# microsoft/ORBIT-Dataset

Measured on AMD Instinct MI355X. Metric: query frames/sec per task (224×224, 5-way ProtoNet) + frame accuracy vs ref, higher is better.
Workload: dtype f32

## Files before the change

### include/orbit_hip.h

```cpp
#ifndef ORBIT_HIP_H
#define ORBIT_HIP_H

#include <stddef.h>
#include <stdint.h>

#ifdef __cplusplus
extern "C" {
#endif

typedef struct orbit_extractor orbit_extractor_t;
typedef struct orbit_filmgen orbit_filmgen_t;
typedef struct orbit_vit orbit_vit_t;
typedef void* orbit_stream_t;

#define ORBIT_OK 0
#define ORBIT_ERR_ARG (-1)
#define ORBIT_ERR_HIP (-2)
#define ORBIT_ERR_STATE (-3)
#define ORBIT_ERR_NOMEM (-4)

#define ORBIT_ACT_NONE 0
#define ORBIT_ACT_RELU 1
#define ORBIT_ACT_SILU 2
#define ORBIT_ACT_ELU 3
// ... 121 lines not shown
int orbit_pw_stream_supported(int Cin, int Cout, int H, int W);
int orbit_op_dwconv2d(const float* x, const float* w, float* y, const float* scale, const float* shift,
                      int B, int H, int W, int C, int K, int stride, int pad_top, int pad_left,
                      int Ho, int Wo, int act, orbit_stream_t stream);
int orbit_op_conv2d_train(const float* x, int x_nchw, const float* w, float* y, const float* gate, int B, int H, int W,
                          int Cin, int Cout, int KH, int KW, int stride, int pad_top, int pad_left, int Ho, int Wo,
                          float* stats, int* stat_blocks, orbit_stream_t stream);
int orbit_op_conv2d_plan(int B, int H, int W, int Cin, int Cout, int KH, int KW, int stride, int pad_top, int pad_left, int Ho, int Wo,
                         int x_nchw, int pool2, int gated, int residual, int flags, int stats_mode, int dual_output, char* row,
                         int* ksplit, int* kt_per_split, int* m_tiles);
int orbit_op_conv2d_plan_ex(int B, int H, int W, int Cin, int Cout, int KH, int KW, int stride, int pad_top, int pad_left, int Ho,
                            int Wo, int x_nchw, int pool2, int gated, int residual, int flags, int stats_mode, int dual_output, int act,
                            char* row, int* ksplit, int* kt_per_split, int* m_tiles, int* epilogue);
int orbit_op_dwconv2d_train(const float* x, const float* w, float* y, const float* in_scale, const float* in_shift,
                            int in_act, int B, int H, int W, int C, int K, int stride, int pad_top, int pad_left, int Ho,
                            int Wo, float* stats, orbit_stream_t stream);
int orbit_op_dwconv2d_se(const float* x, const float* w, const float* scale, const float* shift, int act, int B, int H, int W,
                         int C, int K, int stride, int pad_top, int pad_left, int Ho, int Wo, float* y, float* partial,
                         orbit_stream_t stream);
int orbit_op_dwconv2d_plan(int B, int C, int K, int stride, int Ho, int Wo, int train_form, int* form, int* chunks,
                           int* rows_per_chunk);
int orbit_op_se_gate2(const float* partial, int chunks, int hw, const float* w1, const float* b1, const float* w2,
                      const float* b2, int B, int C, int R, float* gate, float* pooled_out, orbit_stream_t stream);
int orbit_op_maxpool2d(const float* x, float* y, int B, int H, int W, int C, int K, int stride, int pad,
                       int Ho, int Wo, orbit_stream_t stream);
int orbit_op_avgpool(const float* x, float* y, int B, int HW, int C, orbit_stream_t stream);
int orbit_op_se_gate(const float* pooled, const float* w1, const float* b1, const float* w2,
                     const float* b2, float* gate, int B, int C, int R, orbit_stream_t stream);

int orbit_op_vit_linear(const float* x, const float* w, const float* bias, const float* residual, float* y, int M, int N,
                        int K, int epilogue, int tile_rows, orbit_stream_t stream);
int orbit_op_vit_patch_embed(const float* frames, const float* w, const float* bias_or_null, const float* pos_embed,
                             const float* cls_token, float* tokens, int B, int D, int tile_rows, orbit_stream_t stream);
int orbit_op_vit_patch_embed_p(const float* frames, const float* w, const float* bias_or_null, const float* pos_embed,
                               const float* cls_token, float* tokens, int B, int D, int patch, int tile_rows,
                               orbit_stream_t stream);
int orbit_op_vit_layernorm(const float* x, size_t x_stride, float* y, size_t y_stride, int rows, int D, const float* gamma,
                           const float* beta, float eps, orbit_stream_t stream);
int orbit_op_vit_attention(const float* qkv, float* out, int B, int D, int heads, orbit_stream_t stream);
int orbit_op_vit_attention_tokens(const float* qkv, float* out, int B, int tokens, int D, int heads, orbit_stream_t stream);
int orbit_op_vit_linear_dgrad(const float* dy, const float* w, float* wt_scratch, const float* u, const float* residual,
                              float* dx, int M, int N, int K, int tile_rows, orbit_stream_t stream);
int orbit_op_vit_layernorm_bwd(const float* x, size_t x_stride, const float* dy, size_t dy_stride, const float* gamma, float eps,
                               const float* dres, float* dx, size_t dx_stride, int rows, int D, float* dgamma, float* dbeta,
                               float* partial, size_t partial_floats, orbit_stream_t stream);
int orbit_op_vit_attention_bwd(const float* qkv, const float* dout, float* dqkv, int B, int D, int heads,
// ... 278 lines not shown
```

### orbit-dataset_amd/_lib.py

```python
import ctypes
import os
from ctypes import c_char_p, c_double, c_float, c_int, c_size_t, c_void_p, POINTER

_HERE = os.path.dirname(os.path.abspath(__file__))
LIB_PATH = os.path.join(_HERE, "lib", "liborbit_hip.so")

_lib = None

P = c_void_p
_SIGNATURES = {
    "orbit_version": (c_int, []),
    "orbit_last_error": (c_char_p, []),
    "orbit_device_count": (c_int, []),
    "orbit_set_option": (c_int, [c_char_p, c_int]),
    "orbit_get_option": (c_int, [c_char_p]),
    "orbit_label_set": (c_int, [P, c_int, P, c_int, P, P]),
    "orbit_proto_configure": (c_int, [P, P, P, c_int, c_int, c_int, c_int, c_int, P, P, P]),
    "orbit_proto_finalize": (c_int, [P, P, c_int, c_int, c_int, c_int, P, P, P]),
    "orbit_proto_predict": (c_int, [P, P, P, c_int, c_int, c_int, c_int, c_int, c_float, c_int, P, P, P]),
    "orbit_video_metrics": (c_int, [P, c_int, c_int, P, P, c_int, P, P, P, P, P]),
    "orbit_mean_pool": (c_int, [P, c_int, c_int, c_int, P, P]),
    "orbit_set_mean": (c_int, [P, c_int, c_int, P, P]),
    "orbit_history_mean_pool": (c_int, [P, c_int, c_int, c_int, P, P]),
    "orbit_extractor_create": (c_int, [c_char_p, c_int, c_int, POINTER(c_void_p)]),
# ... 38 lines not shown
    "orbit_vit_backward": (c_int, [P, c_int, P, P, P, P, c_size_t, P, P, P, c_size_t, P]),
    "orbit_vit_grad_floats": (c_size_t, [P]),
    "orbit_vit_param_offset": (c_size_t, [P, c_int]),
    "orbit_vit_backward_params_workspace_bytes": (c_size_t, [P, c_int]),
    "orbit_vit_backward_params": (c_int, [P, P, c_int, P, P, P, P, c_size_t, P, P, P, P, c_size_t, P]),
    "orbit_filmgen_create": (c_int, [c_int, c_int, c_int, POINTER(c_int), POINTER(c_int), POINTER(c_int),
                                     POINTER(c_void_p)]),
    "orbit_filmgen_destroy": (None, [P]),
    "orbit_filmgen_load": (c_int, [P, c_int, c_char_p, P, c_size_t]),
    "orbit_filmgen_load_all_async": (c_int, [P, P, c_int, P]),
    "orbit_filmgen_forward": (c_int, [P, P, P, P, P, P]),
    "orbit_op_conv2d": (c_int, [P, c_int, P, P, P, P, P, P] + [c_int] * 14 + [P]),
    "orbit_op_conv2d_ex": (c_int, [P, c_int, P, P, P, P, P, P] + [c_int] * 15 + [P]),
    "orbit_op_dwconv2d": (c_int, [P, P, P, P, P] + [c_int] * 11 + [P]),
    "orbit_op_pw_stream": (c_int, [P] * 6 + [c_int] + [P] * 4 + [c_int, P, P] + [c_int] * 5 + [P]),
    "orbit_pw_stream_supported": (c_int, [c_int] * 4),
    "orbit_op_conv2d_train": (c_int, [P, c_int, P, P, P] + [c_int] * 12 + [P, POINTER(c_int), P]),
    "orbit_op_conv2d_plan": (c_int, [c_int] * 19 + [c_char_p] + [POINTER(c_int)] * 3),
    "orbit_op_conv2d_plan_ex": (c_int, [c_int] * 20 + [c_char_p] + [POINTER(c_int)] * 4),
    "orbit_op_dwconv2d_train": (c_int, [P, P, P, P, P] + [c_int] * 11 + [P, P]),
    "orbit_op_dwconv2d_se": (c_int, [P, P, P, P] + [c_int] * 11 + [P, P, P]),
    "orbit_op_dwconv2d_plan": (c_int, [c_int] * 7 + [POINTER(c_int)] * 3),
    "orbit_op_se_gate2": (c_int, [P, c_int, c_int, P, P, P, P, c_int, c_int, c_int, P, P, P]),
    "orbit_op_maxpool2d": (c_int, [P, P] + [c_int] * 9 + [P]),
    "orbit_op_avgpool": (c_int, [P, P, c_int, c_int, c_int, P]),
    "orbit_op_se_gate": (c_int, [P, P, P, P, P, P, c_int, c_int, c_int, P]),
    "orbit_op_vit_linear": (c_int, [P] * 5 + [c_int] * 5 + [P]),
    "orbit_op_vit_patch_embed": (c_int, [P] * 6 + [c_int] * 3 + [P]),
    "orbit_op_vit_layernorm": (c_int, [P, c_size_t, P, c_size_t, c_int, c_int, P, P, c_float, P]),
    "orbit_op_vit_attention": (c_int, [P, P, c_int, c_int, c_int, P]),
    "orbit_op_vit_attention_tokens": (c_int, [P, P, c_int, c_int, c_int, c_int, P]),
    "orbit_op_vit_patch_embed_p": (c_int, [P] * 6 + [c_int] * 4 + [P]),
    "orbit_op_vit_linear_dgrad": (c_int, [P] * 6 + [c_int] * 4 + [P]),
    "orbit_op_vit_layernorm_bwd": (c_int, [P, c_size_t, P, c_size_t, P, c_float, P, P, c_size_t, c_int, c_int, P, P, P,
                                           c_size_t, P]),
    "orbit_op_vit_attention_bwd": (c_int, [P, P, P, c_int, c_int, c_int, P]),
    "orbit_op_vit_attention_bwd_tokens": (c_int, [P, P, P, c_int, c_int, c_int, c_int, P]),
    "orbit_op_vit_linear_wgrad_workspace_floats": (c_size_t, [c_int, c_int, c_int]),
    "orbit_op_vit_linear_wgrad": (c_int, [P] * 4 + [c_int] * 4 + [P, c_size_t, P]),
    "orbit_op_vit_patch_embed_bwd": (c_int, [P] * 6 + [c_int] * 2 + [P, c_size_t, P]),
    "orbit_op_mbconv_front": (c_int, [P] * 9 + [c_int] * 11 + [P]),
    "orbit_op_mbconv_front_partials": (c_int, [c_int] * 6),
    "orbit_op_stem_dw_front_partials": (c_int, [c_int] * 3),
    "orbit_op_stem_dw_front": (c_int, [P] * 9 + [c_int] * 12 + [P]),
    "orbit_dense_rows": (c_int, [P, c_int, c_int, P, P, c_int, c_int, P, P, P]),
    "orbit_spd_inverse": (c_int, [P, P, c_int, c_int, P]),
# ... 242 lines not shown
```

### orbit-dataset_amd/csrc/common.h

```cpp
#pragma once
#include <hip/hip_runtime.h>
#include <cstdarg>
#include <cstdio>
#include <cstdint>
#include <cstring>
#include <type_traits>
#include "../../include/orbit_hip.h"

namespace orbit {

char* err_buf();
int set_err(int code, const char* fmt, ...);
int get_option(const char* name);
int option_epoch();

#define ORBIT_HIP_CHECK(expr)                                                                  \
    do {                                                                                       \
        hipError_t _e = (expr);                                                                \
        if (_e != hipSuccess)                                                                  \
            return ::orbit::set_err(ORBIT_ERR_HIP, "%s failed: %s (%s:%d)", #expr,             \
                                    hipGetErrorString(_e), __FILE__, __LINE__);                \
    } while (0)

#define ORBIT_LAUNCH_CHECK()                                                                   \
// ... 175 lines not shown
    int form = 0, chunks = 0, rpc = 0, bn_rows = 0, wgrad_rows = 0;
};
DwBwdForm dwconv_se_bwd_form(const LayerGeom& g, bool want_wgrad);
template <class F>
static inline void dw_dispatch_ks(int K, int stride, F&& f) {
    using std::integral_constant;
    if (K == 3 && stride == 1) f(integral_constant<int, 3>{}, integral_constant<int, 1>{});
    else if (K == 3) f(integral_constant<int, 3>{}, integral_constant<int, 2>{});
    else if (stride == 1) f(integral_constant<int, 5>{}, integral_constant<int, 1>{});
    else f(integral_constant<int, 5>{}, integral_constant<int, 2>{});
}
enum DwForm { DW_STREAM, DW_PIPE, DW_WINDOW, DW_LDS };
DwForm dw_form_rule(int K, int stride, int Ho, bool train_form, bool lds_fits = true);
int dwconv_se_chunks(int Ho);
struct DwInXf {
    const float *scale = nullptr, *shift = nullptr;
    int act = ORBIT_ACT_NONE;
};
int launch_dwconv_se(const float* x, const float* w_khwc, float* y, const float* scale, const float* shift,
                     float* pool_partial, const LayerGeom& g, int act, hipStream_t s, int stats = 0, const DwInXf& in = {},
                     const DwBnBwd* bnb = nullptr);
int launch_se_gate2(const float* partial, int chunks, int HW, const float* w1, const float* b1, const float* w2t,
                    const float* b2, float* gate, int B, int C, int R, hipStream_t s, float* pooled_out = nullptr);
int launch_transpose(const float* in, float* out, int rows, int cols, hipStream_t s);
bool stem_direct_supported(int Cin, int Cout, int K, int stride, int W, int act);
int launch_stem_direct(const float* frames, const float* w_oihw, const float* scale, const float* shift, float* y, int B,
                       int H, int W, int pad_t, int pad_l, int Ho, int Wo, hipStream_t s);
bool mbconv_rows_supported(int H, int W, int Cin, int mid, int K, int stride);
int mbconv_rows_tiles(int H, int W, int Cin, int mid, int K, int stride);
int launch_mbconv_rows(const float* x, const float* w1, const float* sc1, const float* sh1, const float* wdw,
                       const float* sc2, const float* sh2, float* y, float* pool, int B, int H, int W, int Cin, int mid,
                       int K, int stride, int pad_t, int pad_l, int Ho, int Wo, hipStream_t s, int plan_tiles = 0,
                       bool raw_stats = false);
bool stem_rows_supported(int H, int W, int mid, int K, int stride);
int stem_rows_tiles(int H, int W);
int launch_stem_rows(const float* frames, const float* w1_packed, const float* sc1, const float* sh1, const float* wdw,
                     const float* sc2, const float* sh2, float* y, float* pool, int B, int FH, int FW, int spad_t,
                     int spad_l, int H, int W, hipStream_t s, int plan_tiles = 0);
int stem_pack_weights(const float* w_oihw, float* w_packed, int mid, hipStream_t s);
int dwconv_pack_weights(const float* w, float* w_khwc, int C, int K, hipStream_t s);
int launch_maxpool(const float* x, float* y, const LayerGeom& g, hipStream_t s);
int launch_avgpool(const float* x, float* y, int B, int HW, int C, hipStream_t s);
int launch_se_gate(const float* pooled, const float* w1, const float* b1, const float* w2,
                   const float* b2, float* gate, int B, int C, int R, hipStream_t s);


// ... 94 lines not shown
```

### orbit-dataset_amd/csrc/extractor.hip

```cpp
#include <chrono>
#include <cstdlib>

#include "extractor.h"

using namespace orbit;

static int conv_out(int H, int K, int stride, int pad) { return (H + 2 * pad - K) / stride + 1; }
static void same_pad(int H, int K, int stride, int& Ho, int& pad_before) {
    Ho = (H + stride - 1) / stride;
    const int total = std::max((Ho - 1) * stride + K - H, 0);
    pad_before = total / 2;
}

static int build_resnet18(orbit_extractor* fe, int H, int W) {
    fe->out_size = 512;
    int h = conv_out(H, 7, 2, 3), w = conv_out(W, 7, 2, 3);
    int bn = fe->add_bn("bn1", 64, 1e-5f, true);
    fe->add_conv("conv1.weight", bn, -1, 0, -1, H, W, 3, 64, 7, 2, 3, 3, h, w, ORBIT_ACT_RELU, 0, 1, 0);
    {
        Op o;
        o.kind = OP_MAXPOOL, o.in = 0, o.out = 1, o.H = h, o.W = w, o.Cin = 64, o.Cout = 64;
        o.pool_k = 3, o.stride = 2, o.pool_pad = 1;
        o.Ho = conv_out(h, 3, 2, 1), o.Wo = conv_out(w, 3, 2, 1);
        h = o.Ho, w = o.Wo;
// ... 464 lines not shown
                          (double)(fe->ops.size() + 1);
        fe->eager_us_per_launch = fe->eager_samples == 0 ? us : 0.7 * fe->eager_us_per_launch + 0.3 * us;
        fe->eager_samples++;
        return rc;
    }

    orbit_extractor::GraphKey key;
    memset(&key, 0, sizeof(key));
    key.frames = frames, key.gamma = film_gamma, key.beta = film_beta, key.feats = feats, key.ws = workspace, key.B = B;
    bool replayed = false;
    return fe->graphs.run(
        key, s, &fe->cap_stream,
        [&](hipStream_t rs) { return run_plan(fe, frames, B, film_gamma, film_beta, feats, workspace, rs); }, &replayed);
}

static bool se_in_projection(const orbit_extractor_t* fe, size_t i) {
    if (!get_option("conv_rgemm") || i + 1 >= fe->ops.size() || fe->ops[i].kind != OP_SE) return false;
    const Op& c = fe->ops[i + 1];
    return c.kind == OP_CONV && c.use_gate && c.Cin == fe->ops[i].Cin && c.KH == 1 && c.KW == 1 && c.stride == 1 &&
           c.pad_t == 0 && c.pad_l == 0 && !c.x_nchw && !c.pool2 && c.act == ORBIT_ACT_NONE && c.bn >= 0 &&
           c.Ho == c.H && c.Wo == c.W && pw_stream_supported(c.Cin, c.Cout, c.H, c.W);
}

enum ServedBy {
    BY_OWN_LAUNCHER,
    BY_STEM_DIRECT,
    BY_PW_STREAM,
    BY_PROJECTION
};
static ServedBy served_by(const orbit_extractor_t* fe, size_t oi, ServedBy prev) {
    const Op& o = fe->ops[oi];
    if (o.kind == OP_SE) return se_in_projection(fe, oi) ? BY_PROJECTION : BY_OWN_LAUNCHER;
    if (o.kind != OP_CONV) return BY_OWN_LAUNCHER;
    if (o.x_nchw && !o.pool2 && o.res < 0 && o.bn >= 0 && stem_direct_supported(o.Cin, o.Cout, o.KH, o.stride, o.W, o.act) &&
        o.KH == o.KW)
        return BY_STEM_DIRECT;
    return prev == BY_PROJECTION ? BY_PW_STREAM : BY_OWN_LAUNCHER;
}

static int run_plan(orbit_extractor_t* fe, const float* frames, int B, const float* film_gamma, const float* film_beta,
                    float* feats, void* workspace, hipStream_t s) {
    const WsLayout L = ws_layout(fe, B);
    char* ws = static_cast<char*>(workspace);
    auto buf = [&](int id) -> float* {
        if (id == -1) return const_cast<float*>(frames);
        if (id == BUF_FEATS) return feats;
        if (id == BUF_POOLED) return reinterpret_cast<float*>(ws + L.pooled);
        if (id == BUF_GATE) return reinterpret_cast<float*>(ws + L.gate);
        return reinterpret_cast<float*>(ws + L.buf[id]);
    };
    const float* scale = fe->d_fold;
    const float* shift = fe->d_fold + fe->fold_floats;
    if (film_gamma && fe->film_size > 0) {
        float* fs = reinterpret_cast<float*>(ws + L.fold);
        dim3 grid((unsigned)fe->bns.size(), 2);
// ... 22 lines not shown
                    d.x = buf(o.in), d.w_packed = fe->d_packed + o.packed_off, d.y = buf(o.out);
                    d.scale = scale + fe->bns[o.bn].fold_off, d.shift = shift + fe->bns[o.bn].fold_off;
                    d.residual = o.res >= 0 ? buf(o.res) : nullptr;
                    d.partial = buf(BUF_POOLED), d.chunks = se.se_chunks, d.se_hw = se.se_hw;
                    d.w1 = fe->param(se.se_w1), d.b1 = fe->param(se.se_b1);
                    d.w2t = fe->d_packed + se.packed_off, d.b2 = fe->param(se.se_b2), d.R = se.R;
                    d.B = B, d.H = o.H, d.W = o.W, d.Cin = o.Cin, d.Cout = o.Cout;
                    rc = launch_pw_stream(d, s);
                    break;
                }
                ConvDesc d = o.conv_desc(B);
                d.x = buf(o.in), d.w_packed = fe->d_packed + o.packed_off, d.y = buf(o.out);
                d.w_frag = o.frag_off != SIZE_MAX ? fe->d_packed + o.frag_off : nullptr;
                d.scale = o.bn >= 0 ? scale + fe->bns[o.bn].fold_off : nullptr;
                d.shift = o.bn >= 0 ? shift + fe->bns[o.bn].fold_off : nullptr;
                d.residual = o.res >= 0 ? buf(o.res) : nullptr;
                d.gate = o.use_gate ? buf(BUF_GATE) : nullptr;
                d.splitk_ws = reinterpret_cast<float*>(ws + L.splitk);
                d.lean_epilogue = true;
                rc = launch_conv(d, s);
                break;
            }
            case OP_DWCONV:
                rc = launch_dwconv_se(buf(o.in), fe->d_packed + o.packed_off, buf(o.out),
                                      scale + fe->bns[o.bn].fold_off, shift + fe->bns[o.bn].fold_off,
                                      o.pool_partial ? buf(BUF_POOLED) : nullptr, o.geom(B), o.act, s);
                break;
            case OP_MBFRONT:
                if (o.stem)
                    rc = launch_stem_rows(buf(o.in), fe->d_packed + o.packed_off2, scale + fe->bns[o.bn].fold_off,
                                          shift + fe->bns[o.bn].fold_off, fe->d_packed + o.packed_off,
                                          scale + fe->bns[o.bn2].fold_off, shift + fe->bns[o.bn2].fold_off, buf(o.out),
                                          buf(BUF_POOLED), B, o.stem_h, o.stem_w, o.stem_pt, o.stem_pl, o.H, o.W, s, o.se_chunks);
                else
                    rc = launch_mbconv_rows(buf(o.in), fe->param(o.weight),
                                            scale + fe->bns[o.bn].fold_off, shift + fe->bns[o.bn].fold_off,
                                            fe->d_packed + o.packed_off, scale + fe->bns[o.bn2].fold_off,
                                            shift + fe->bns[o.bn2].fold_off, buf(o.out), buf(BUF_POOLED), B, o.H, o.W, o.Cin,
                                            o.Cout, o.KH, o.stride, o.pad_t, o.pad_l, o.Ho, o.Wo, s, o.se_chunks);
                break;
            case OP_MAXPOOL:
                rc = launch_maxpool(buf(o.in), buf(o.out), o.geom(B), s);
                break;
            case OP_AVGPOOL:
                rc = launch_avgpool(buf(o.in), buf(o.out), B, o.H * o.W, o.Cin, s);
                break;
            case OP_SE:
                if (by == BY_PROJECTION) break;
                rc = launch_se_gate2(buf(BUF_POOLED), o.se_chunks, o.se_hw, fe->param(o.se_w1),
                                     fe->param(o.se_b1), fe->d_packed + o.packed_off,
                                     fe->param(o.se_b2), buf(BUF_GATE), B, o.Cin, o.R, s);
                break;
        }
        if (rc != ORBIT_OK) return rc;
    }
    return ORBIT_OK;
}

}
```

### orbit-dataset_amd/csrc/ops.hip

```cpp
#include "common.h"
#include "device_util.h"
#include "se_gate.h"
#include <algorithm>

namespace orbit {

using v4f = __attribute__((ext_vector_type(4))) float;

struct DwBnbVec {
    v4f sc, sh, mu, is;
};
__device__ __forceinline__ v4f dw_bnb(v4f dx, v4f yv, const DwBnbVec& b, int act, v4f& s0, v4f& s1) {
    const v4f z = yv * b.sc + b.sh;
    v4f g = dx;
    if (act == ORBIT_ACT_SILU) {
#pragma unroll
        for (int k = 0; k < 4; ++k) {
            const float sg = __builtin_amdgcn_rcpf(1.0f + __expf(-z[k]));
            g[k] *= sg * (1.0f + z[k] * (1.0f - sg));
        }
    } else if (act == ORBIT_ACT_RELU) {
#pragma unroll
        for (int k = 0; k < 4; ++k) g[k] = z[k] > 0.f ? g[k] : 0.f;
    }
// ... 392 lines not shown
            for (int l = 1; l < WL; ++l) t += red[l * cb4 + tid];
            *reinterpret_cast<v4f*>(pool_partial + (prow + 1) * C + (c4_0 + tid) * 4) = t;
        }
    }
    if (WG) {
        v4f* wred = wl + K * K * cb4;
        constexpr int TB = 8;
        const size_t wrow = (size_t)b * gridDim.y + chunk;
#pragma unroll
        for (int t0 = 0; t0 < K * K; t0 += TB) {
            __syncthreads();
#pragma unroll
            for (int u = 0; u < TB; ++u)
                if (t0 + u < K * K) wred[u * 256 + tid] = active ? wacc[t0 + u] : (v4f){0.f, 0.f, 0.f, 0.f};
            __syncthreads();
            for (int i = tid; i < TB * cb4; i += 256) {
                const int u = i / cb4, cc = i - u * cb4;
                if (t0 + u < K * K) {
                    v4f t = wred[u * 256 + cc];
                    for (int l = 1; l < WL; ++l) t += wred[u * 256 + l * cb4 + cc];
                    *reinterpret_cast<v4f*>(bnb.wgrad_partial + (wrow * K * K + (K * K - 1 - (t0 + u))) * C + (c4_0 + cc) * 4) = t;
                }
            }
        }
    }
}

template <int K, int S, int U, bool STATS = false, bool XF = false, bool BNB = false>
__global__ __launch_bounds__(256) void dwconv_lds_kernel(const float* __restrict__ x, const float* __restrict__ w,
                                                         float* __restrict__ y, const float* __restrict__ scale,
                                                         const float* __restrict__ shift,
                                                         float* __restrict__ pool_partial, int H, int W, int C,
                                                         int pad_t, int pad_l, int Ho, int Wo, int act, int cs4,
                                                         int rows_per_chunk, int G, int IWA,
                                                         DwInXf xf = DwInXf{nullptr, nullptr, 0}, DwBnBwd bnb = DwBnBwd{}) {
    constexpr int NCOL = 3 * S + K;
    extern __shared__ __attribute__((aligned(16))) float sml[];
    const int CSP = cs4 * 4 + 4;
    const int b = blockIdx.z, chunk = blockIdx.y;
    const int c0 = blockIdx.x * cs4 * 4;
    const int ho0 = chunk * rows_per_chunk;
    const int TH = min(Ho, ho0 + rows_per_chunk) - ho0;
    const int IH = (TH - 1) * S + K;
    const int IHmax = (rows_per_chunk - 1) * S + K;
    float* tile = sml;
    v4f* wl = reinterpret_cast<v4f*>(sml + (size_t)IHmax * IWA * CSP);
// ... 35 lines not shown
#pragma unroll
            for (int u = 0; u < U; ++u)
                if (dst[u] >= 0)
                    *reinterpret_cast<v4f*>(tile + dst[u]) = (XF && ((loaded >> u) & 1u)) ? dw_xf(v[u], xsc, xsh, xf.act) : v[u];
        }
    }
#pragma unroll
    for (int u = 0; u < 2; ++u)
        if (tid + u * 256 < K * K * cs4) wl[tid + u * 256] = wq[u];
    __syncthreads();
    v4f sc = {1.f, 1.f, 1.f, 1.f}, sh = {0.f, 0.f, 0.f, 0.f}, psum = {0.f, 0.f, 0.f, 0.f}, psq = {0.f, 0.f, 0.f, 0.f};
    if (scale) sc = *reinterpret_cast<const v4f*>(scale + c);
    if (shift) sh = *reinterpret_cast<const v4f*>(shift + c);
    const int RL = P / G;
    const int g = p % G, rl = p / G;
    float* yb = y + (size_t)b * Ho * Wo * C + c;
    DwBnbVec bv;
    const float* byb = nullptr;
    if (BNB) {
        bv.sc = *reinterpret_cast<const v4f*>(bnb.bn.scale + c), bv.sh = *reinterpret_cast<const v4f*>(bnb.bn.shift + c);
        bv.mu = *reinterpret_cast<const v4f*>(bnb.bn.mean + c), bv.is = *reinterpret_cast<const v4f*>(bnb.bn.invstd + c);
        byb = bnb.y + (size_t)b * Ho * Wo * C + c;
    }
    if (rl < RL) {
        for (int ro = rl; ro < TH; ro += RL) {
            v4f acc[4];
#pragma unroll
            for (int j = 0; j < 4; ++j) acc[j] = (v4f){0.f, 0.f, 0.f, 0.f};
            const float* t0 = tile + ((size_t)(ro * S) * IWA + g * 4 * S) * CSP + lc * 4;
            const v4f* wk = wl + lc;
            const int ho = ho0 + ro;
            v4f yv[4];
            if (BNB) {
#pragma unroll
                for (int j = 0; j < 4; ++j)
                    yv[j] = *reinterpret_cast<const v4f*>(byb + ((size_t)ho * Wo + min(g * 4 + j, Wo - 1)) * C);
            }
#pragma unroll 1
            for (int kh = 0; kh < K; ++kh) {
                v4f col[NCOL];
#pragma unroll
                for (int q = 0; q < NCOL; ++q) col[q] = *reinterpret_cast<const v4f*>(t0 + q * CSP);
#pragma unroll
                for (int kw = 0; kw < K; ++kw) {
                    const v4f f = wk[kw * cs4];
#pragma unroll
                    for (int j = 0; j < 4; ++j) acc[j] += col[j * S + kw] * f;
                }
                t0 += IWA * CSP;
                wk += K * cs4;
            }
#pragma unroll
            for (int j = 0; j < 4; ++j) {
                const int wo = g * 4 + j;
                if (wo < Wo) {
                    if (BNB) {
                        *reinterpret_cast<v4f*>(yb + ((size_t)ho * Wo + wo) * C) = dw_bnb(acc[j], yv[j], bv, bnb.act, psum, psq);
                    } else {
                        v4f o = acc[j] * sc + sh;
                        o[0] = apply_act(o[0], act), o[1] = apply_act(o[1], act), o[2] = apply_act(o[2], act), o[3] = apply_act(o[3], act);
                        *reinterpret_cast<v4f*>(yb + ((size_t)ho * Wo + wo) * C) = o;
                        psum += o;
                        if (STATS) psq += o * o;
                    }
                }
            }
        }
    }
    if (pool_partial == nullptr) return;
    red[p * cs4 + lc] = psum;
    __syncthreads();
    const size_t prow = ((size_t)b * gridDim.y + chunk) * (STATS ? 2 : 1);
    if (tid < cs4) {
        v4f t = red[tid];
        for (int l = 1; l < P; ++l) t += red[l * cs4 + tid];
        *reinterpret_cast<v4f*>(pool_partial + prow * C + c0 + tid * 4) = t;
    }
    if (STATS) {
        __syncthreads();
        red[p * cs4 + lc] = psq;
        __syncthreads();
        if (tid < cs4) {
            v4f t = red[tid];
            for (int l = 1; l < P; ++l) t += red[l * cs4 + tid];
            *reinterpret_cast<v4f*>(pool_partial + (prow + 1) * C + c0 + tid * 4) = t;
        }
    }
}

template <int NT>
__global__ __launch_bounds__(NT) void se_gate2_kernel(const float* __restrict__ partial, int chunks, float inv_hw,
                                                       const float* __restrict__ w1, const float* __restrict__ b1,
                                                       const float* __restrict__ w2t, const float* __restrict__ b2,
                                                       float* __restrict__ gate, int C, int R,
                                                       float* __restrict__ pooled_out) {
    extern __shared__ __attribute__((aligned(16))) float sm2[];
    const int b = blockIdx.x;
    se_gate_frame<NT, 4>(partial + (size_t)b * chunks * C, chunks, inv_hw, w1, b1, w2t, b2, gate + (size_t)b * C, C, R,
                         pooled_out ? pooled_out + (size_t)b * C : nullptr, sm2);
}

__global__ __launch_bounds__(256) void transpose_kernel(const float* __restrict__ in, float* __restrict__ out, int rows,
                                                        int cols) {
    const int total = rows * cols;
    for (int i = blockIdx.x * 256 + threadIdx.x; i < total; i += gridDim.x * 256) {
        const int r = i / cols, c = i % cols;
        out[(size_t)c * rows + r] = in[i];
    }
}

// ... 61 lines not shown
    __syncthreads();
    for (int c = threadIdx.x; c < C; c += 256) {
        float s = b2[c];
        for (int r = 0; r < R; ++r) s = fmaf(w2[(size_t)c * R + r], hid[r], s);
        gate[(size_t)b * C + c] = 1.0f / (1.0f + expf(-s));
    }
}

static int grid_for(size_t total) {
    size_t b = (total + 255) / 256;
    return (int)(b > 8192 ? 8192 : (b == 0 ? 1 : b));
}

static int dw_cb4(int C) {
    const int c4 = C / 4;
    for (int d = c4 < 64 ? c4 : 64; d >= 1; --d)
        if (c4 % d == 0) return d;
    return 1;
}
static int dwconv_se_rows_per_chunk(int Ho) { return Ho >= 56 ? 8 : (Ho >= 14 ? 7 : Ho); }
int dwconv_se_chunks(int Ho) { return cdiv(Ho, dwconv_se_rows_per_chunk(Ho)); }

DwForm dw_form_rule(int K, int stride, int Ho, bool train_form, bool lds_fits) {
    const int lds_opt = get_option("dw_lds");
    if (lds_fits && (lds_opt == 2 || (lds_opt == 1 && ((stride == 1 && (K == 5 || Ho <= 14)) || (train_form && stride == 2 && Ho < 14)))))
        return DW_LDS;
    const int win_opt = get_option("dw_window");
    if (win_opt == 2 || (win_opt == 1 && K == 3 && stride == 1 && Ho >= 14)) return DW_WINDOW;
    const int pipe_opt = get_option("dw_pipe");
    if (pipe_opt == 2 || (pipe_opt == 1 && stride == 2 && Ho >= (train_form ? 14 : 28))) return DW_PIPE;
    return DW_STREAM;
}

bool dwconv_se_window_form(int K, int stride, int Ho) { return dw_form_rule(K, stride, Ho, false) == DW_WINDOW; }

struct DwPlan {
    DwForm form;
    int cb4, rpc;
    dim3 grid;
    size_t lds;
    int cs4, G, IWA;
    bool deep;
};
static DwPlan dw_plan(int B, int C, int K, int stride, int Ho, int Wo, bool train_form) {
    DwPlan p{};
    p.cb4 = dw_cb4(C), p.rpc = dwconv_se_rows_per_chunk(Ho);
    p.form = dw_form_rule(K, stride, Ho, train_form);
    if (p.form == DW_LDS) {
        const int c4 = C / 4;
        p.G = cdiv(Wo, 4);
        for (int cand : {16, 8, 4}) {
            if (c4 % cand != 0 || p.G > 256 / cand) continue;
            p.cs4 = cand;
            if (2 * ((256 / cand) / p.G) >= p.rpc) break;
        }
        p.IWA = (4 * p.G - 1) * stride + K;
        const int IHmax = (p.rpc - 1) * stride + K;
        p.lds = ((size_t)IHmax * p.IWA * (p.cs4 * 4 + 4)) * sizeof(float) + (size_t)(K * K * p.cs4 + 256) * sizeof(float4);
        if (p.cs4 != 0 && p.lds <= 64 * 1024) {
            p.grid = dim3(c4 / p.cs4, cdiv(Ho, p.rpc), B);
            p.deep = IHmax * p.IWA > 8 * (256 / p.cs4);
            return p;
        }
        p.form = dw_form_rule(K, stride, Ho, train_form, false);
    }
    p.grid = dim3(C / 4 / p.cb4, cdiv(Ho, p.rpc), B);
    p.lds = (size_t)(K * K * p.cb4 + (256 / p.cb4) * p.cb4) * sizeof(float4);
    return p;
}

static DwBwdForm dw_bwd_form(const DwPlan& p, int stride, bool want_wgrad) {
    DwBwdForm f;
    f.form = p.form, f.chunks = (int)p.grid.y, f.rpc = p.rpc;
    const int rows = (int)(p.grid.y * p.grid.z);
    if (stride == 1 && (p.form == DW_LDS || p.form == DW_WINDOW)) f.bn_rows = rows;
    if (stride == 1 && p.form == DW_WINDOW && want_wgrad) f.wgrad_rows = rows;
    return f;
}
DwBwdForm dwconv_se_bwd_form(const LayerGeom& g, bool want_wgrad) {
    return dw_bwd_form(dw_plan(g.B, g.Cin, g.KH, g.stride, g.Ho, g.Wo, false), g.stride, want_wgrad);
}

static int launch_dwconv_se_impl(const float* x, const float* w_khwc, float* y, const float* scale, const float* shift,
                                 float* pool_partial, const LayerGeom& g, int act, hipStream_t s, int stats, const DwInXf& xf,
                                 const DwBnBwd* bnb);

int launch_dwconv_se(const float* x, const float* w_khwc, float* y, const float* scale, const float* shift,
                     float* pool_partial, const LayerGeom& g, int act, hipStream_t s, int stats, const DwInXf& in, const DwBnBwd* bnb) {
    int rec = -1;
    if (conv_prof_enabled()) {
        const int C = g.Cin, K = g.KH;
// ... 104 lines not shown
                                                                cb4, rpc);
            break;
        }
    });
    ORBIT_LAUNCH_CHECK();
    return ORBIT_OK;
}

int launch_se_gate2(const float* partial, int chunks, int HW, const float* w1, const float* b1, const float* w2t,
                    const float* b2, float* gate, int B, int C, int R, hipStream_t s, float* pooled_out) {
    ORBIT_REQUIRE(partial && w1 && b1 && w2t && b2 && gate, "se_gate2: null pointer");
    ORBIT_REQUIRE(C % 4 == 0, "se_gate2: C %% 4 != 0 (C=%d)", C);
    const size_t lds = (size_t)(((C + R + 3) & ~3) + 4 * 1024) * sizeof(float);
    const int rec = prof_start("se_gate", 4.0 * B * C * R, 4.0 * ((double)B * chunks * C + 2.0 * C * R + C + R + (double)B * C), s);
    if (C >= 1024)
        se_gate2_kernel<1024><<<B, 1024, lds, s>>>(partial, chunks, 1.0f / (float)HW, w1, b1, w2t, b2, gate, C, R, pooled_out);
    else
        se_gate2_kernel<256><<<B, 256, lds, s>>>(partial, chunks, 1.0f / (float)HW, w1, b1, w2t, b2, gate, C, R, pooled_out);
    prof_stop(rec, s);
    ORBIT_LAUNCH_CHECK();
    return ORBIT_OK;
}

int launch_transpose(const float* in, float* out, int rows, int cols, hipStream_t s) {
    transpose_kernel<<<grid_for((size_t)rows * cols), 256, 0, s>>>(in, out, rows, cols);
    ORBIT_LAUNCH_CHECK();
    return ORBIT_OK;
}

int dwconv_pack_weights(const float* w, float* w_khwc, int C, int K, hipStream_t s) {
    dw_pack_kernel<<<grid_for((size_t)C * K * K), 256, 0, s>>>(w, w_khwc, C, K);
    ORBIT_LAUNCH_CHECK();
    return ORBIT_OK;
}

int launch_maxpool(const float* x, float* y, const LayerGeom& g, hipStream_t s) {
    const int B = g.B, H = g.H, W = g.W, C = g.Cin, K = g.KH, stride = g.stride, pad = g.pad_t, Ho = g.Ho, Wo = g.Wo;
    ORBIT_REQUIRE(x && y, "maxpool: null pointer");
    ORBIT_REQUIRE(C % 4 == 0, "maxpool: C %% 4 != 0 (C=%d)", C);
    const size_t total = (size_t)B * Ho * Wo * (C / 4);
    ORBIT_REQUIRE(total < (1ull << 32), "maxpool: tensor too large for 32-bit index arithmetic");
    const int rec = prof_start("maxpool", 0.0, 4.0 * ((double)B * H * W * C + (double)B * Ho * Wo * C), s);
    maxpool_kernel<<<grid_for(total), 256, 0, s>>>(x, y, B, H, W, C, K, stride, pad, Ho, Wo);
    prof_stop(rec, s);
    ORBIT_LAUNCH_CHECK();
    return ORBIT_OK;
// ... 75 lines not shown
int orbit_op_dwconv2d_plan(int B, int C, int K, int stride, int Ho, int Wo, int train_form, int* form, int* chunks,
                           int* rows_per_chunk) {
    ORBIT_REQUIRE(form && chunks && rows_per_chunk, "op_dwconv2d_plan: null pointer");
    ORBIT_REQUIRE(B > 0 && C > 0 && C % 4 == 0 && Ho > 0 && Wo > 0 && (K == 3 || K == 5) && (stride == 1 || stride == 2),
                  "op_dwconv2d_plan: bad geometry");
    const DwPlan p = dw_plan(B, C, K, stride, Ho, Wo, train_form != 0);
    *form = (int)p.form, *chunks = (int)p.grid.y, *rows_per_chunk = p.rpc;
    return ORBIT_OK;
}

int orbit_op_se_gate2(const float* partial, int chunks, int hw, const float* w1, const float* b1, const float* w2,
                      const float* b2, int B, int C, int R, float* gate, float* pooled_out, orbit_stream_t stream) {
    ORBIT_REQUIRE(partial && w1 && b1 && w2 && b2 && gate, "op_se_gate2: null pointer");
    ORBIT_REQUIRE(B > 0 && C > 0 && R > 0 && chunks > 0 && hw > 0, "op_se_gate2: bad sizes");
    hipStream_t s = (hipStream_t)stream;
    float* w2t = nullptr;
    ORBIT_HIP_CHECK(hipMallocAsync(reinterpret_cast<void**>(&w2t), (size_t)C * R * sizeof(float), s));
    int rc = launch_transpose(w2, w2t, C, R, s);
    if (rc == ORBIT_OK) rc = launch_se_gate2(partial, chunks, hw, w1, b1, w2t, b2, gate, B, C, R, s, pooled_out);
    (void)hipFreeAsync(w2t, s);
    return rc;
}

int orbit_op_maxpool2d(const float* x, float* y, int B, int H, int W, int C, int K, int stride, int pad,
                       int Ho, int Wo, orbit_stream_t stream) {
    return launch_maxpool(x, y, LayerGeom{B, H, W, C, C, K, K, stride, pad, pad, Ho, Wo}, (hipStream_t)stream);
}

int orbit_op_avgpool(const float* x, float* y, int B, int HW, int C, orbit_stream_t stream) {
    return launch_avgpool(x, y, B, HW, C, (hipStream_t)stream);
}

int orbit_op_se_gate(const float* pooled, const float* w1, const float* b1, const float* w2, const float* b2,
                     float* gate, int B, int C, int R, orbit_stream_t stream) {
    return launch_se_gate(pooled, w1, b1, w2, b2, gate, B, C, R, (hipStream_t)stream);
}

}
```

Measured before the change: 38200.

## Fuse depthwise conv and SE gate into one per-frame kernel for 7x7 layers

Adds a kernel that runs one block per frame for small (at most 7x7, stride 1) depthwise layers followed by squeeze-excitation. Each wave stages channel slices in LDS with register double-buffered prefetch, computes the depthwise output plus pooled sums, and the block then computes the SE gate in place. This replaces the separate dwconv and se_gate2 launches, removing a launch and the pooled-partial round trip through global memory. The trade-off is that only B blocks run with large LDS use, so small batches may underuse the GPU. The shared row loop is pulled out into a helper.

New measurement: 38160. Within noise of the previous version (-0.1%).

```diff
diff --git a/include/orbit_hip.h b/include/orbit_hip.h
--- a/include/orbit_hip.h
+++ b/include/orbit_hip.h
@@ -167,6 +167,11 @@
                            int* rows_per_chunk);
 int orbit_op_se_gate2(const float* partial, int chunks, int hw, const float* w1, const float* b1, const float* w2,
                       const float* b2, int B, int C, int R, float* gate, float* pooled_out, orbit_stream_t stream);
+int orbit_op_dw_frame_plan(int B, int C, int K, int stride, int Ho, int Wo, int R, int* applies, int* threads, int* slices_in_flight,
+                           int* lds_bytes);
+int orbit_op_dwconv2d_se_gate_frame(const float* x, const float* w, const float* scale, const float* shift, int act, int B, int H,
+                                    int W, int C, int K, int pad_top, int pad_left, int Ho, int Wo, const float* w1, const float* b1,
+                                    const float* w2, const float* b2, int R, float* y, float* gate, orbit_stream_t stream);
 int orbit_op_maxpool2d(const float* x, float* y, int B, int H, int W, int C, int K, int stride, int pad,
                        int Ho, int Wo, orbit_stream_t stream);
 int orbit_op_avgpool(const float* x, float* y, int B, int HW, int C, orbit_stream_t stream);
diff --git a/orbit-dataset_amd/_lib.py b/orbit-dataset_amd/_lib.py
--- a/orbit-dataset_amd/_lib.py
+++ b/orbit-dataset_amd/_lib.py
@@ -84,6 +84,8 @@
     "orbit_op_dwconv2d_se": (c_int, [P, P, P, P] + [c_int] * 11 + [P, P, P]),
     "orbit_op_dwconv2d_plan": (c_int, [c_int] * 7 + [POINTER(c_int)] * 3),
     "orbit_op_se_gate2": (c_int, [P, c_int, c_int, P, P, P, P, c_int, c_int, c_int, P, P, P]),
+    "orbit_op_dw_frame_plan": (c_int, [c_int] * 7 + [POINTER(c_int)] * 4),
+    "orbit_op_dwconv2d_se_gate_frame": (c_int, [P, P, P, P] + [c_int] * 10 + [P, P, P, P, c_int, P, P, P]),
     "orbit_op_maxpool2d": (c_int, [P, P] + [c_int] * 9 + [P]),
     "orbit_op_avgpool": (c_int, [P, P, c_int, c_int, c_int, P]),
     "orbit_op_se_gate": (c_int, [P, P, P, P, P, P, c_int, c_int, c_int, P]),
diff --git a/orbit-dataset_amd/csrc/common.h b/orbit-dataset_amd/csrc/common.h
--- a/orbit-dataset_amd/csrc/common.h
+++ b/orbit-dataset_amd/csrc/common.h
@@ -221,6 +221,17 @@
                      const DwBnBwd* bnb = nullptr);
 int launch_se_gate2(const float* partial, int chunks, int HW, const float* w1, const float* b1, const float* w2t,
                     const float* b2, float* gate, int B, int C, int R, hipStream_t s, float* pooled_out = nullptr);
+struct DwFramePlan {
+    bool applies;
+    int threads, groups;
+    int cs4, G, IWA;
+    int grp_floats, pooled_off;
+    size_t lds;
+};
+DwFramePlan dw_frame_plan(int B, int C, int K, int stride, int Ho, int Wo, int R);
+int launch_dwconv_frame_gate(const float* x, const float* w_khwc, float* y, const float* scale, const float* shift,
+                             const LayerGeom& g, int act, const float* w1, const float* b1, const float* w2t, const float* b2, int R,
+                             float* gate, hipStream_t s);
 int launch_transpose(const float* in, float* out, int rows, int cols, hipStream_t s);
 bool stem_direct_supported(int Cin, int Cout, int K, int stride, int W, int act);
 int launch_stem_direct(const float* frames, const float* w_oihw, const float* scale, const float* shift, float* y, int B,
diff --git a/orbit-dataset_amd/csrc/extractor.hip b/orbit-dataset_amd/csrc/extractor.hip
--- a/orbit-dataset_amd/csrc/extractor.hip
+++ b/orbit-dataset_amd/csrc/extractor.hip
@@ -510,15 +510,25 @@
            c.Ho == c.H && c.Wo == c.W && pw_stream_supported(c.Cin, c.Cout, c.H, c.W);
 }
 
+static bool dw_with_gate(const orbit_extractor_t* fe, size_t i) {
+    if (i + 1 >= fe->ops.size() || fe->ops[i].kind != OP_DWCONV || !fe->ops[i].pool_partial || fe->ops[i].bn < 0) return false;
+    const Op &d = fe->ops[i], &se = fe->ops[i + 1];
+    return se.kind == OP_SE && se.Cin == d.Cin && se.se_chunks == 1 && se.se_hw == d.Ho * d.Wo && d.KH == d.KW &&
+           !se_in_projection(fe, i + 1) && dw_frame_plan(1, d.Cin, d.KH, d.stride, d.Ho, d.Wo, se.R).applies;
+}
+
 enum ServedBy {
     BY_OWN_LAUNCHER,
     BY_STEM_DIRECT,
     BY_PW_STREAM,
-    BY_PROJECTION
+    BY_PROJECTION,
+    BY_FRAME_GATE,
+    BY_DEPTHWISE
 };
 static ServedBy served_by(const orbit_extractor_t* fe, size_t oi, ServedBy prev) {
     const Op& o = fe->ops[oi];
-    if (o.kind == OP_SE) return se_in_projection(fe, oi) ? BY_PROJECTION : BY_OWN_LAUNCHER;
+    if (o.kind == OP_DWCONV) return dw_with_gate(fe, oi) ? BY_FRAME_GATE : BY_OWN_LAUNCHER;
+    if (o.kind == OP_SE) return prev == BY_FRAME_GATE ? BY_DEPTHWISE : (se_in_projection(fe, oi) ? BY_PROJECTION : BY_OWN_LAUNCHER);
     if (o.kind != OP_CONV) return BY_OWN_LAUNCHER;
     if (o.x_nchw && !o.pool2 && o.res < 0 && o.bn >= 0 && stem_direct_supported(o.Cin, o.Cout, o.KH, o.stride, o.W, o.act) &&
         o.KH == o.KW)
@@ -587,6 +597,14 @@
                 break;
             }
             case OP_DWCONV:
+                if (by == BY_FRAME_GATE) {
+                    const Op& se = fe->ops[oi + 1];
+                    rc = launch_dwconv_frame_gate(buf(o.in), fe->d_packed + o.packed_off, buf(o.out), scale + fe->bns[o.bn].fold_off,
+                                                  shift + fe->bns[o.bn].fold_off, o.geom(B), o.act, fe->param(se.se_w1),
+                                                  fe->param(se.se_b1), fe->d_packed + se.packed_off, fe->param(se.se_b2), se.R,
+                                                  buf(BUF_GATE), s);
+                    break;
+                }
                 rc = launch_dwconv_se(buf(o.in), fe->d_packed + o.packed_off, buf(o.out),
                                       scale + fe->bns[o.bn].fold_off, shift + fe->bns[o.bn].fold_off,
                                       o.pool_partial ? buf(BUF_POOLED) : nullptr, o.geom(B), o.act, s);
@@ -612,6 +630,7 @@
                 break;
             case OP_SE:
                 if (by == BY_PROJECTION) break;
+                if (by == BY_DEPTHWISE) break;
                 rc = launch_se_gate2(buf(BUF_POOLED), o.se_chunks, o.se_hw, fe->param(o.se_w1),
                                      fe->param(o.se_b1), fe->d_packed + o.packed_off,
                                      fe->param(o.se_b2), buf(BUF_GATE), B, o.Cin, o.R, s);
diff --git a/orbit-dataset_amd/csrc/ops.hip b/orbit-dataset_amd/csrc/ops.hip
--- a/orbit-dataset_amd/csrc/ops.hip
+++ b/orbit-dataset_amd/csrc/ops.hip
@@ -438,6 +438,59 @@
                     *reinterpret_cast<v4f*>(bnb.wgrad_partial + (wrow * K * K + (K * K - 1 - (t0 + u))) * C + (c4_0 + cc) * 4) = t;
                 }
             }
+        }
+    }
+}
+
+template <int K, int S, bool STATS, bool BNB, bool ONE = false>
+__device__ __forceinline__ void dw_lds_rows(const float* tile, const v4f* wl, float* __restrict__ yb, const float* __restrict__ byb,
+                                            const DwBnbVec& bv, int bnb_act, v4f sc, v4f sh, int act, int lc, int g, int rl, int RL,
+                                            int TH, int ho0, int RPF, int CSP, int cs4, int Wo, int C, v4f& psum, v4f& psq) {
+    constexpr int NCOL = 3 * S + K;
+    if (rl < RL) {
+        for (int ro = rl; ro < TH; ro += RL) {
+            v4f acc[4];
+#pragma unroll
+            for (int j = 0; j < 4; ++j) acc[j] = (v4f){0.f, 0.f, 0.f, 0.f};
+            const float* t0 = tile + (size_t)(ro * S) * RPF + (size_t)(g * 4 * S) * CSP + lc * 4;
+            const v4f* wk = wl + lc;
+            const int ho = ho0 + ro;
+            v4f yv[4];
+            if (BNB) {
+#pragma unroll
+                for (int j = 0; j < 4; ++j)
+                    yv[j] = *reinterpret_cast<const v4f*>(byb + ((size_t)ho * Wo + min(g * 4 + j, Wo - 1)) * C);
+            }
+#pragma unroll 1
+            for (int kh = 0; kh < K; ++kh) {
+                v4f col[NCOL];
+#pragma unroll
+                for (int q = 0; q < NCOL; ++q) col[q] = *reinterpret_cast<const v4f*>(t0 + q * CSP);
+#pragma unroll
+                for (int kw = 0; kw < K; ++kw) {
+                    const v4f f = wk[kw * cs4];
+#pragma unroll
+                    for (int j = 0; j < 4; ++j) acc[j] += col[j * S + kw] * f;
+                }
+                t0 += RPF;
+                wk += K * cs4;
+            }
+#pragma unroll
+            for (int j = 0; j < 4; ++j) {
+                const int wo = g * 4 + j;
+                if (wo < Wo) {
+                    if (BNB) {
+                        *reinterpret_cast<v4f*>(yb + ((size_t)ho * Wo + wo) * C) = dw_bnb(acc[j], yv[j], bv, bnb_act, psum, psq);
+                    } else {
+                        v4f o = acc[j] * sc + sh;
+                        o[0] = apply_act(o[0], act), o[1] = apply_act(o[1], act), o[2] = apply_act(o[2], act), o[3] = apply_act(o[3], act);
+                        *reinterpret_cast<v4f*>(yb + ((size_t)ho * Wo + wo) * C) = o;
+                        psum += o;
+                        if (STATS) psq += o * o;
+                    }
+                }
+            }
+            if (ONE) break;
         }
     }
 }
@@ -519,51 +572,7 @@
         bv.mu = *reinterpret_cast<const v4f*>(bnb.bn.mean + c), bv.is = *reinterpret_cast<const v4f*>(bnb.bn.invstd + c);
         byb = bnb.y + (size_t)b * Ho * Wo * C + c;
     }
-    if (rl < RL) {
-        for (int ro = rl; ro < TH; ro += RL) {
-            v4f acc[4];
-#pragma unroll
-            for (int j = 0; j < 4; ++j) acc[j] = (v4f){0.f, 0.f, 0.f, 0.f};
-            const float* t0 = tile + ((size_t)(ro * S) * IWA + g * 4 * S) * CSP + lc * 4;
-            const v4f* wk = wl + lc;
-            const int ho = ho0 + ro;
-            v4f yv[4];
-            if (BNB) {
-#pragma unroll
-                for (int j = 0; j < 4; ++j)
-                    yv[j] = *reinterpret_cast<const v4f*>(byb + ((size_t)ho * Wo + min(g * 4 + j, Wo - 1)) * C);
-            }
-#pragma unroll 1
-            for (int kh = 0; kh < K; ++kh) {
-                v4f col[NCOL];
-#pragma unroll
-                for (int q = 0; q < NCOL; ++q) col[q] = *reinterpret_cast<const v4f*>(t0 + q * CSP);
-#pragma unroll
-                for (int kw = 0; kw < K; ++kw) {
-                    const v4f f = wk[kw * cs4];
-#pragma unroll
-                    for (int j = 0; j < 4; ++j) acc[j] += col[j * S + kw] * f;
-                }
-                t0 += IWA * CSP;
-                wk += K * cs4;
-            }
-#pragma unroll
-            for (int j = 0; j < 4; ++j) {
-                const int wo = g * 4 + j;
-                if (wo < Wo) {
-                    if (BNB) {
-                        *reinterpret_cast<v4f*>(yb + ((size_t)ho * Wo + wo) * C) = dw_bnb(acc[j], yv[j], bv, bnb.act, psum, psq);
-                    } else {
-                        v4f o = acc[j] * sc + sh;
-                        o[0] = apply_act(o[0], act), o[1] = apply_act(o[1], act), o[2] = apply_act(o[2], act), o[3] = apply_act(o[3], act);
-                        *reinterpret_cast<v4f*>(yb + ((size_t)ho * Wo + wo) * C) = o;
-                        psum += o;
-                        if (STATS) psq += o * o;
-                    }
-                }
-            }
-        }
-    }
+    dw_lds_rows<K, S, STATS, BNB>(tile, wl, yb, byb, bv, bnb.act, sc, sh, act, lc, g, rl, RL, TH, ho0, IWA * CSP, CSP, cs4, Wo, C, psum, psq);
     if (pool_partial == nullptr) return;
     red[p * cs4 + lc] = psum;
     __syncthreads();
@@ -583,6 +592,108 @@
             *reinterpret_cast<v4f*>(pool_partial + (prow + 1) * C + c0 + tid * 4) = t;
         }
     }
+}
+
+
+__host__ __device__ inline int dwf_row_floats(int IWA) { return 4 * (IWA * 4 + ((4 - IWA * 4) & 15)); }
+constexpr int DWF_WAVES = 8, DWF_CS4 = 4, DWF_ITEMS = 9, DWF_GATE_U = 6;
+__device__ __forceinline__ void wave_lds_sync() {
+    __builtin_amdgcn_fence(__ATOMIC_RELEASE, "wavefront");
+    __builtin_amdgcn_wave_barrier();
+    __builtin_amdgcn_fence(__ATOMIC_ACQUIRE, "wavefront");
+}
+template <int K, int NW>
+__global__ __launch_bounds__(64 * NW) void dwconv_frame_gate_kernel(
+    const float* __restrict__ x, const float* __restrict__ w, float* __restrict__ y, const float* __restrict__ scale,
+    const float* __restrict__ shift, const float* __restrict__ w1, const float* __restrict__ b1, const float* __restrict__ w2t,
+    const float* __restrict__ b2, float* __restrict__ gate, int H, int W, int C, int pad_t, int pad_l, int Ho, int Wo, int act, int G,
+    int IWA, int R, float inv_hw, int grp_floats, int pooled_off) {
+    constexpr int cs4 = DWF_CS4, CSP = cs4 * 4, P = 64 / cs4;
+    const int RPF = dwf_row_floats(IWA);
+    extern __shared__ __attribute__((aligned(16))) float smf[];
+    const int IH = Ho - 1 + K, n_items = IH * IWA;
+    const int b = blockIdx.x;
+    const int wave = __builtin_amdgcn_readfirstlane(threadIdx.x >> 6), tid = threadIdx.x & 63;
+    float* tile = smf + (size_t)wave * grp_floats;
+    v4f* wl = reinterpret_cast<v4f*>(tile + (size_t)IH * RPF);
+    v4f* red = wl + K * K * cs4;
+    v4f* pooled4 = reinterpret_cast<v4f*>(smf + pooled_off);
+    const int lc = tid % cs4, p = tid / cs4;
+    const int RL = P / G, g = p % G, rl = p / G;
+    const int nsl = (C >> 2) / cs4;
+    const float* xf = x + (size_t)b * H * W * C;
+    float* yf = y + (size_t)b * Ho * Wo * C;
+    int poff[DWF_ITEMS], pdst[DWF_ITEMS], woff[2];
+    unsigned inside = 0;
+    {
+        const int dr = P / IWA, dc = P % IWA;
+        int r = p / IWA, col = p % IWA;
+#pragma unroll
+        for (int u = 0; u < DWF_ITEMS; ++u) {
+            const int hi = r - pad_t, wi = col - pad_l;
+            const bool in = p + u * P < n_items && (unsigned)hi < (unsigned)H && (unsigned)wi < (unsigned)W;
+            poff[u] = in ? (hi * W + wi) * C + lc * 4 : lc * 4;
+            pdst[u] = r * RPF + col * CSP + lc * 4;
+            inside |= in ? 1u << u : 0u;
+            r += dr, col += dc;
+            if (col >= IWA) col -= IWA, ++r;
+        }
+#pragma unroll
+        for (int u = 0; u < 2; ++u) {
+            const int i = tid + u * 64;
+            woff[u] = i < K * K * cs4 ? (i / cs4) * C + (i % cs4) * 4 : 0;
+        }
+    }
+    struct SliceRegs {
+        v4f pv[DWF_ITEMS], wq[2], sc, sh;
+    };
+    auto load_slice = [&](int sl, SliceRegs& r) {
+        const int c0 = sl * cs4 * 4;
+#pragma unroll
+        for (int u = 0; u < 2; ++u) r.wq[u] = *reinterpret_cast<const v4f*>(w + c0 + woff[u]);
+#pragma unroll
+        for (int u = 0; u < DWF_ITEMS; ++u) r.pv[u] = *reinterpret_cast<const v4f*>(xf + c0 + poff[u]);
+        r.sc = *reinterpret_cast<const v4f*>(scale + c0 + lc * 4);
+        r.sh = *reinterpret_cast<const v4f*>(shift + c0 + lc * 4);
+    };
+    auto run_slice = [&](int sl, SliceRegs& r, bool valid) {
+        v4f sc = {1.f, 1.f, 1.f, 1.f}, sh = {0.f, 0.f, 0.f, 0.f};
+        if (valid) {
+#pragma unroll
+            for (int u = 0; u < DWF_ITEMS; ++u)
+                if (p + u * P < n_items)
+                    *reinterpret_cast<v4f*>(tile + pdst[u]) = (inside >> u) & 1u ? r.pv[u] : (v4f){0.f, 0.f, 0.f, 0.f};
+#pragma unroll
+            for (int u = 0; u < 2; ++u)
+                if (tid + u * 64 < K * K * cs4) wl[tid + u * 64] = r.wq[u];
+            sc = r.sc, sh = r.sh;
+            wave_lds_sync();
+        }
+        load_slice(min(sl + 2 * NW, nsl - 1), r);
+        if (valid) {
+            v4f psum = {0.f, 0.f, 0.f, 0.f}, psq = {0.f, 0.f, 0.f, 0.f};
+            const DwBnbVec no_bnb{};
+            dw_lds_rows<K, 1, false, false, true>(tile, wl, yf + sl * cs4 * 4 + lc * 4, nullptr, no_bnb, 0, sc, sh, act, lc, g, rl, RL, Ho, 0, RPF,
+                                            CSP, cs4, Wo, C, psum, psq);
+            red[p * cs4 + lc] = psum;
+            wave_lds_sync();
+            if (tid < cs4) {
+                v4f t = red[tid];
+                for (int l = 1; l < P; ++l) t += red[l * cs4 + tid];
+                pooled4[sl * cs4 + tid] = t;
+            }
+            wave_lds_sync();
+        }
+    };
+    SliceRegs ra, rb;
+    load_slice(min(wave, nsl - 1), ra);
+    load_slice(min(wave + NW, nsl - 1), rb);
+    for (int sl = wave; sl < nsl; sl += 2 * NW) {
+        run_slice(sl, ra, true);
+        run_slice(sl + NW, rb, sl + NW < nsl);
+    }
+    __syncthreads();
+    se_gate_frame<64 * NW, DWF_GATE_U>(smf + pooled_off, 1, inv_hw, w1, b1, w2t, b2, gate + (size_t)b * C, C, R, nullptr, smf);
 }
 
 template <int NT>
@@ -690,7 +801,8 @@
 int dwconv_se_chunks(int Ho) { return cdiv(Ho, dwconv_se_rows_per_chunk(Ho)); }
 
 DwForm dw_form_rule(int K, int stride, int Ho, bool train_form, bool lds_fits) {
-    const int lds_opt = get_option("dw_lds");
+    const int lds_raw = get_option("dw_lds");
+    const int lds_opt = lds_raw == 3 ? 1 : lds_raw;
     if (lds_fits && (lds_opt == 2 || (lds_opt == 1 && ((stride == 1 && (K == 5 || Ho <= 14)) || (train_form && stride == 2 && Ho < 14)))))
         return DW_LDS;
     const int win_opt = get_option("dw_window");
@@ -735,6 +847,27 @@
     p.grid = dim3(C / 4 / p.cb4, cdiv(Ho, p.rpc), B);
     p.lds = (size_t)(K * K * p.cb4 + (256 / p.cb4) * p.cb4) * sizeof(float4);
     return p;
+}
+
+constexpr size_t DWF_LDS_MAX = 112 * 1024;
+DwFramePlan dw_frame_plan(int B, int C, int K, int stride, int Ho, int Wo, int R) {
+    DwFramePlan f{};
+    const int opt = get_option("dw_lds");
+    if (opt == 3 || (opt != 2 && C > 1152)) return f;
+    if (B <= 0 || C <= 0 || C % 4 != 0 || R <= 0 || (K != 3 && K != 5) || stride != 1 || Ho <= 0 || Wo <= 0 || Ho > 7 || Wo > 7) return f;
+    const DwPlan p = dw_plan(B, C, K, 1, Ho, Wo, false);
+    if (p.form != DW_LDS || p.grid.y != 1) return f;
+    if ((C / 4) % DWF_CS4 != 0 || 64 / DWF_CS4 < p.G) return f;
+    f.groups = DWF_WAVES, f.threads = 64 * DWF_WAVES;
+    f.cs4 = DWF_CS4, f.G = p.G, f.IWA = p.IWA;
+    const int n_items = (Ho - 1 + K) * p.IWA;
+    if (n_items > DWF_ITEMS * (64 / DWF_CS4) || K * K * DWF_CS4 > 128 || (64 / DWF_CS4) / p.G < Ho) return f;
+    f.grp_floats = (Ho - 1 + K) * dwf_row_floats(p.IWA) + 4 * (K * K * DWF_CS4) + 4 * 64;
+    const int gate_floats = ((C + R + 3) & ~3) + 4 * f.threads;
+    f.pooled_off = std::max(f.groups * f.grp_floats, gate_floats);
+    f.lds = (size_t)(f.pooled_off + C) * sizeof(float);
+    f.applies = f.lds <= DWF_LDS_MAX;
+    return f;
 }
 
 static DwBwdForm dw_bwd_form(const DwPlan& p, int stride, bool want_wgrad) {
@@ -885,6 +1018,45 @@
     return ORBIT_OK;
 }
 
+int launch_dwconv_frame_gate(const float* x, const float* w_khwc, float* y, const float* scale, const float* shift,
+                             const LayerGeom& g, int act, const float* w1, const float* b1, const float* w2t, const float* b2, int R,
+                             float* gate, hipStream_t s) {
+    const int B = g.B, C = g.Cin, K = g.KH;
+    ORBIT_REQUIRE(x && w_khwc && y && scale && shift && w1 && b1 && w2t && b2 && gate, "dwconv_frame_gate: null pointer");
+    const DwFramePlan f = dw_frame_plan(B, C, K, g.stride, g.Ho, g.Wo, R);
+    ORBIT_REQUIRE(f.applies, "dwconv_frame_gate: the per-frame form does not apply (C=%d K=%d stride=%d %dx%d R=%d)", C, K, g.stride,
+                  g.Ho, g.Wo, R);
+    int rec = -1;
+    if (conv_prof_enabled()) {
+        char name[48];
+        snprintf(name, sizeof(name), "dwconv_frame_gate<%d>", K);
+        const double out = (double)B * g.Ho * g.Wo * C;
+        rec = prof_start(name, 2.0 * out * K * K + 4.0 * B * C * R,
+                         4.0 * ((double)B * g.H * g.W * C + out + (double)K * K * C + 2.0 * C * R + C + R + (double)B * C), s,
+                         act == ORBIT_ACT_SILU ? out : 0.0);
+    }
+    const float inv_hw = 1.0f / (float)(g.Ho * g.Wo);
+    static bool attr_set = false;
+    if (!attr_set) {
+        ORBIT_HIP_CHECK(hipFuncSetAttribute(reinterpret_cast<const void*>(dwconv_frame_gate_kernel<3, DWF_WAVES>),
+                                            hipFuncAttributeMaxDynamicSharedMemorySize, (int)DWF_LDS_MAX));
+        ORBIT_HIP_CHECK(hipFuncSetAttribute(reinterpret_cast<const void*>(dwconv_frame_gate_kernel<5, DWF_WAVES>),
+                                            hipFuncAttributeMaxDynamicSharedMemorySize, (int)DWF_LDS_MAX));
+        attr_set = true;
+    }
+    if (K == 3)
+        dwconv_frame_gate_kernel<3, DWF_WAVES><<<B, f.threads, f.lds, s>>>(x, w_khwc, y, scale, shift, w1, b1, w2t, b2, gate, g.H, g.W, C,
+                                                                        g.pad_t, g.pad_l, g.Ho, g.Wo, act, f.G, f.IWA, R, inv_hw,
+                                                                        f.grp_floats, f.pooled_off);
+    else
+        dwconv_frame_gate_kernel<5, DWF_WAVES><<<B, f.threads, f.lds, s>>>(x, w_khwc, y, scale, shift, w1, b1, w2t, b2, gate, g.H, g.W, C,
+                                                                        g.pad_t, g.pad_l, g.Ho, g.Wo, act, f.G, f.IWA, R, inv_hw,
+                                                                        f.grp_floats, f.pooled_off);
+    prof_stop(rec, s);
+    ORBIT_LAUNCH_CHECK();
+    return ORBIT_OK;
+}
+
 int launch_transpose(const float* in, float* out, int rows, int cols, hipStream_t s) {
     transpose_kernel<<<grid_for((size_t)rows * cols), 256, 0, s>>>(in, out, rows, cols);
     ORBIT_LAUNCH_CHECK();
@@ -1006,6 +1178,35 @@
     return rc;
 }
 
+int orbit_op_dw_frame_plan(int B, int C, int K, int stride, int Ho, int Wo, int R, int* applies, int* threads, int* slices_in_flight,
+                           int* lds_bytes) {
+    ORBIT_REQUIRE(applies && threads && slices_in_flight && lds_bytes, "op_dw_frame_plan: null pointer");
+    const DwFramePlan f = dw_frame_plan(B, C, K, stride, Ho, Wo, R);
+    *applies = f.applies ? 1 : 0;
+    *threads = f.applies ? f.threads : 0, *slices_in_flight = f.applies ? f.groups : 0, *lds_bytes = f.applies ? (int)f.lds : 0;
+    return ORBIT_OK;
+}
+
+int orbit_op_dwconv2d_se_gate_frame(const float* x, const float* w, const float* scale, const float* shift, int act, int B, int H,
+                                    int W, int C, int K, int pad_top, int pad_left, int Ho, int Wo, const float* w1, const float* b1,
+                                    const float* w2, const float* b2, int R, float* y, float* gate, orbit_stream_t stream) {
+    ORBIT_REQUIRE(x && w && scale && shift && y && gate && w1 && b1 && w2 && b2, "op_dwconv2d_se_gate_frame: null pointer");
+    ORBIT_REQUIRE(B > 0 && C > 0 && R > 0 && H > 0 && W > 0 && Ho > 0 && Wo > 0 && (K == 3 || K == 5),
+                  "op_dwconv2d_se_gate_frame: bad geometry");
+    ORBIT_REQUIRE(dw_frame_plan(B, C, K, 1, Ho, Wo, R).applies, "op_dwconv2d_se_gate_frame: the per-frame form does not apply");
+    hipStream_t s = (hipStream_t)stream;
+    float* tmp = nullptr;
+    const size_t wfl = ((size_t)C * K * K + 63) & ~(size_t)63;
+    ORBIT_HIP_CHECK(hipMallocAsync(reinterpret_cast<void**>(&tmp), (wfl + (size_t)C * R) * sizeof(float), s));
+    int rc = dwconv_pack_weights(w, tmp, C, K, s);
+    if (rc == ORBIT_OK) rc = launch_transpose(w2, tmp + wfl, C, R, s);
+    if (rc == ORBIT_OK)
+        rc = launch_dwconv_frame_gate(x, tmp, y, scale, shift, LayerGeom{B, H, W, C, C, K, K, 1, pad_top, pad_left, Ho, Wo}, act, w1, b1,
+                                      tmp + wfl, b2, R, gate, s);
+    (void)hipFreeAsync(tmp, s);
+    return rc;
+}
+
 int orbit_op_maxpool2d(const float* x, float* y, int B, int H, int W, int C, int K, int stride, int pad,
                        int Ho, int Wo, orbit_stream_t stream) {
     return launch_maxpool(x, y, LayerGeom{B, H, W, C, C, K, K, stride, pad, pad, Ho, Wo}, (hipStream_t)stream);
```
